# GabrieleConte/pokemon-sprite-generator

Measured on AMD Instinct MI355X. Metric: unet_train_steps_per_sec_bs256, higher is better.
Workload: dtype bf16; 1 GPU; full train_step (add_noise+fwd+SmoothL1+bwd+clip+AdamW), U-Net 640M params, per-GPU batch 256, 27x27x8 latents, 32x256 text, 8 heads, train mode (dropout 0.05), bf16 MFMA / fp32 master+accum; per_gpu_batch=256, global_batch=256, parallelism=dp1

## Files before the change

### include/psg_hip.h

```cpp
#ifndef PSG_HIP_H
#define PSG_HIP_H

#include <stdint.h>

#ifdef __cplusplus
extern "C" {
#endif

typedef void* psg_stream_t;

enum psg_status {
    PSG_OK = 0,
    PSG_ERR_SHAPE = -1,
    PSG_ERR_DTYPE = -2,
    PSG_ERR_ALIGN = -3,
    PSG_ERR_WORKSPACE = -4,
    PSG_ERR_HIP = -5,
    PSG_ERR_ARG = -6
};
enum psg_dtype { PSG_F32 = 0, PSG_BF16 = 1 };
enum psg_act { PSG_ACT_NONE = 0, PSG_ACT_SILU = 1, PSG_ACT_GELU = 2, PSG_ACT_RELU = 3, PSG_ACT_TANH = 4 };
enum psg_flag {
    PSG_FLAG_NOISY_BAD = 1,
    PSG_FLAG_T_RANGE = 2,
    PSG_FLAG_PRED_BAD = 4,
    PSG_FLAG_LOSS_BAD = 8,
    PSG_FLAG_FALLBACK = 16,
    PSG_FLAG_INPUT_BAD = 32,
    PSG_FLAG_SKIP_MASK = 47
};

const char* psg_last_error(void);
int psg_version(void);
// ... 140 lines not shown
int psg_attn_route(int pass, int dtype, int B, int heads, int L, int S, int d, int64_t ldq, int64_t ldk, int64_t ldv,
                   int64_t ldo, int64_t ld_grads, int ptrs_aligned16, int32_t* out);
int psg_attn_bwd(const void* q, int64_t ldq, const void* k, int64_t ldk, const void* v, int64_t ldv,
                 const void* o, int64_t ldo, const void* dout, int64_t lddo, const float* lse,
                 float* delta, void* dq, int64_t lddq, void* dk, int64_t lddk, void* dv, int64_t lddv,
                 int B, int heads, int L, int S, int d, float scale, float drop_p, uint64_t seed,
                 int dtype, psg_stream_t stream);

int psg_attn_bwd_longq(const void* q, int64_t ldq, const void* k, int64_t ldk, const void* v, int64_t ldv,
                       const void* o, int64_t ldo, const void* dout, int64_t lddo, const float* lse,
                       float* delta, void* dq, int64_t lddq, void* dk, int64_t lddk, void* dv, int64_t lddv,
                       int B, int heads, int L, int S, int d, float scale, float drop_p, uint64_t seed,
                       int dtype, void* ws, int64_t ws_bytes, psg_stream_t stream);
int64_t psg_attn_bwd_longq_workspace_bytes(int B, int heads, int L, int S, int d);

int psg_attn_bwd_varlen(const void* q, int64_t ldq, const void* k, int64_t ldk, const void* v, int64_t ldv,
                        const void* o, int64_t ldo, const void* dout, int64_t lddo, const float* lse,
                        float* delta, void* dq, int64_t lddq, void* dk, int64_t lddk, void* dv, int64_t lddv,
                        int B, int heads, int L, int S, int d, float scale, float drop_p, uint64_t seed,
                        int dtype, const int32_t* kv_len, psg_stream_t stream);

int psg_layernorm(const void* x, int64_t ldx, const void* r, int64_t ldr, void* y, int64_t ldy, const float* gamma,
                  const float* beta, int64_t rows, int N, float eps, int x_dtype, int y_dtype, psg_stream_t stream);
int psg_layernorm_bwd(const void* x, int64_t ldx, const void* r, int64_t ldr, const void* dy, int64_t lddy,
                      const float* gamma, void* dz, int64_t lddz, float* dgamma, float* dbeta, int accumulate,
                      int64_t rows, int N, float eps, int x_dtype, int dy_dtype, void* ws, int64_t ws_bytes,
                      psg_stream_t stream);
int64_t psg_layernorm_bwd_workspace_bytes(int64_t rows, int N);
int psg_bert_embed_ln(const int64_t* ids, const int64_t* type_ids, const float* word_emb, const float* pos_emb,
                      const float* type_emb, const float* gamma, const float* beta, void* y, int64_t ldy, int B, int S,
// ... 31 lines not shown
```

### pokemon_sprite_generator_amd/_lib.py

```python
import ctypes as C
import os

import torch

_HERE = os.path.dirname(os.path.abspath(__file__))
LIB_PATH = os.environ.get("PSG_LIB_PATH") or os.path.join(_HERE, "libpsg_hip.so")

PSG_F32, PSG_BF16 = 0, 1
ACT_NONE, ACT_SILU, ACT_GELU, ACT_RELU, ACT_TANH = 0, 1, 2, 3, 4
CONV_SAVE_DACT, CONV_DACT_MUL, CONV_GENERIC_EPILOGUE = 1, 2, 4
FLAG_NOISY_BAD, FLAG_T_RANGE, FLAG_PRED_BAD, FLAG_LOSS_BAD, FLAG_FALLBACK, FLAG_INPUT_BAD, FLAG_SKIP_MASK = 1, 2, 4, 8, 16, 32, 47

c_void_p, c_int, c_int64, c_float, c_uint64 = C.c_void_p, C.c_int, C.c_int64, C.c_float, C.c_uint64


class ConvDesc(C.Structure):
    _fields_ = [
        ("dtype", C.c_int32), ("B", C.c_int32), ("Hi", C.c_int32), ("Wi", C.c_int32), ("Cin", C.c_int32),
        ("Ho", C.c_int32), ("Wo", C.c_int32), ("Cout", C.c_int32),
        ("ksize", C.c_int32), ("stride", C.c_int32), ("pad", C.c_int32),
        ("transposed", C.c_int32), ("act", C.c_int32),
        ("alpha", C.c_float), ("drop_p", C.c_float), ("flags", C.c_int32), ("drop_seed", C.c_uint64),
        ("ldx", C.c_int64), ("ldy", C.c_int64), ("ld_rowadd", C.c_int64), ("ld_residual", C.c_int64),
        ("ld_preact", C.c_int64), ("ld_dact", C.c_int64), ("ldw", C.c_int64),
# ... 60 lines not shown
                                 c_uint64, c_int, c_void_p]),
    "psg_dropout_apply": (c_int, [c_void_p, c_int64, c_void_p, c_int64, c_int64, c_int, c_float, c_uint64, c_float, c_int, c_void_p]),
    "psg_attn_fwd": (c_int, [c_void_p, c_int64, c_void_p, c_int64, c_void_p, c_int64, c_void_p, c_int64, c_void_p]
                     + [c_int] * 5 + [c_float, c_float, c_uint64, c_int, c_void_p]),
    "psg_attn_fwd_varlen": (c_int, [c_void_p, c_int64, c_void_p, c_int64, c_void_p, c_int64, c_void_p, c_int64, c_void_p]
                            + [c_int] * 5 + [c_float, c_float, c_uint64, c_int, c_void_p, c_void_p]),
    "psg_attn_fwd_varlen_train": (c_int, [c_void_p, c_int64, c_void_p, c_int64, c_void_p, c_int64, c_void_p, c_int64, c_void_p]
                                  + [c_int] * 5 + [c_float, c_float, c_uint64, c_int, c_void_p, c_void_p]),
    "psg_attn_bwd_varlen": (c_int, [c_void_p, c_int64] * 5 + [c_void_p, c_void_p] + [c_void_p, c_int64] * 3
                            + [c_int] * 5 + [c_float, c_float, c_uint64, c_int, c_void_p, c_void_p]),
    "psg_attn_path_counts": (c_int, [c_void_p, c_void_p, c_void_p]),
    "psg_attn_set_paths": (c_int, [c_int]),
    "psg_attn_route": (c_int, [c_int] * 7 + [c_int64] * 5 + [c_int, c_void_p]),
    "psg_attn_bwd": (c_int, [c_void_p, c_int64] * 5 + [c_void_p, c_void_p] + [c_void_p, c_int64] * 3
                     + [c_int] * 5 + [c_float, c_float, c_uint64, c_int, c_void_p]),
    "psg_attn_bwd_longq": (c_int, [c_void_p, c_int64] * 5 + [c_void_p, c_void_p] + [c_void_p, c_int64] * 3
                           + [c_int] * 5 + [c_float, c_float, c_uint64, c_int, c_void_p, c_int64, c_void_p]),
    "psg_attn_bwd_longq_workspace_bytes": (c_int64, [c_int] * 5),
    "psg_recon_loss_f32": (c_int, [c_void_p] * 4 + [c_int64, c_float, c_float, c_void_p, c_void_p]),
    "psg_recon_loss_workspace_bytes": (c_int64, []),
    "psg_layernorm": (c_int, [c_void_p, c_int64, c_void_p, c_int64, c_void_p, c_int64, c_void_p, c_void_p, c_int64, c_int, c_float,
                              c_int, c_int, c_void_p]),
    "psg_layernorm_bwd": (c_int, [c_void_p, c_int64, c_void_p, c_int64, c_void_p, c_int64, c_void_p, c_void_p, c_int64, c_void_p, c_void_p,
                                  c_int, c_int64, c_int, c_float, c_int, c_int, c_void_p, c_int64, c_void_p]),
    "psg_layernorm_bwd_workspace_bytes": (c_int64, [c_int64, c_int]),
    "psg_bert_embed_ln": (c_int, [c_void_p] * 8 + [c_int64] + [c_int] * 6 + [c_float, c_int, c_void_p]),
    "psg_sumsq_f32": (c_int, [c_void_p, c_int64, c_void_p, c_int, c_void_p, c_void_p]),
    "psg_adamw_f32": (c_int, [c_void_p] * 4 + [c_int64] + [c_float] * 5 + [c_int, c_void_p, c_float, c_void_p, c_void_p, c_void_p]),
    "psg_adamw_dev_f32": (c_int, [c_void_p] * 4 + [c_int64, c_void_p, c_void_p, c_int] + [c_float] * 4 + [c_void_p, c_void_p, c_float, c_void_p, c_void_p, c_void_p]),
    "psg_clip_scale_f32": (c_int, [c_void_p, c_int64, c_void_p, c_float, c_void_p]),
# ... 146 lines not shown
```

### pokemon_sprite_generator_amd/csrc/attention.h

```cpp
#pragma once
#include "psg_common.h"

namespace psg {

template <typename T>
struct AttnArgs {
    const T *q, *k, *v, *o, *dout;
    T *out, *dq, *dk, *dv;
    float* lse; float* delta;
    int64_t ldq, ldk, ldv, ldo, lddo, lddq, lddk, lddv;
    int B, H, L, S, d;
    float scale;
    uint32_t drop_thresh; float drop_scale; uint64_t seed;
    const uint64_t* seed_dev;
    const int32_t* kv_len;
};

template <typename NDs, typename F>
inline bool with_nd(NDs nds, int d, F&& f) { return d % 16 == 0 && with_const(nds, d / 16, f); }
template <int... NDs, typename F>
inline int for_each_nd(std::integer_sequence<int, NDs...>, F&& f) {
    int rc = PSG_OK;
    ((rc = rc ? rc : f(std::integral_constant<int, NDs>{})), ...);
    return rc;
// ... 3 lines not shown
    int nd;
    int waves;
    int kw, qw, dkv_waves;
    int qw_cut, w_cut;
    int nh, kv_reg;
    size_t lds_fwd, lds_dq, lds_dkv;
    int grid_q[2], grid_kv[2];
};

bool attn_mfma_applicable(int L, int S, int d, int64_t ldq, int64_t ldk, int64_t ldv, int64_t ldo, bool forward_only);
AttnPlan attn_mfma_plan(int B, int H, int L, int S, int d);
int attn_mfma_init_attrs();
template <bool VARLEN> int attn_mfma_fwd(const AttnArgs<bf16_t>& p, hipStream_t s);
template <bool VARLEN> int attn_mfma_bwd(const AttnArgs<bf16_t>& p, hipStream_t s);

bool attn_f32_applicable(int L, int S, int d, int64_t ldq, int64_t ldk, int64_t ldv, int64_t ldo, bool forward_only);
AttnPlan attn_f32_plan(int B, int H, int L, int S, int d);
int attn_f32_init_attrs();
template <bool VARLEN> int attn_f32_fwd(const AttnArgs<float>& p, hipStream_t s);
template <bool VARLEN> int attn_f32_bwd(const AttnArgs<float>& p, hipStream_t s);

int attn_longq_init_attrs();

}
```

### pokemon_sprite_generator_amd/csrc/attention.hip

```cpp
#include "attention.h"
#include <type_traits>

namespace psg {

constexpr int AT_Q = 16;
constexpr int AT_KC = 32;
constexpr int AT_MAXC = 20;

template <typename T>
__device__ __forceinline__ uint64_t attn_idx(const AttnArgs<T>& p, int bh, int l, int s) {
    return ((uint64_t)bh * p.L + l) * (uint64_t)(2 * ((p.S + 1) >> 1)) + s;
}

template <typename T>
__device__ __forceinline__ void stage_rows(float* dst, const T* base, int64_t ld, int r0, int rows, int rmax, int d, float scl) {
    const int d4 = d >> 2;
    for (int e = threadIdx.x; e < rows * d4; e += blockDim.x) {
        const int r = e / d4, c = (e - r * d4) * 4;
        f32x4 v = {0.f, 0.f, 0.f, 0.f};
        if (r0 + r < rmax) v = load4<T>(base + (int64_t)(r0 + r) * ld + c);
        float* o = dst + r * (d + 1) + c;
        o[0] = v[0] * scl; o[1] = v[1] * scl; o[2] = v[2] * scl; o[3] = v[3] * scl;
    }
}
// ... 414 lines not shown
        }
        PSG_LAUNCH_CHECK("attn_bwd");
    } else if (varlen) {
        hipLaunchKernelGGL((attn_fwd_kernel<T, true>), grid, block, pl.lds_fwd, s, p);
        PSG_LAUNCH_CHECK("attn_fwd_varlen");
    } else {
        hipLaunchKernelGGL((attn_fwd_kernel<T, false>), grid, block, pl.lds_fwd, s, p);
        PSG_LAUNCH_CHECK("attn_fwd");
    }
    return PSG_OK;
}

template <typename F>
static int with_elem(int dtype, F&& f) { return dtype == PSG_BF16 ? f((bf16_t*)nullptr) : f((float*)nullptr); }

static int attn_bwd_entry(const char* who, const int32_t* kv_len, const void* q, int64_t ldq, const void* k, int64_t ldk, const void* v, int64_t ldv, const void* o,
                 int64_t ldo, const void* dout, int64_t lddo, const float* lse, float* delta, void* dq, int64_t lddq,
                 void* dk, int64_t lddk, void* dv, int64_t lddv, int B, int heads, int L, int S, int d, float scale,
                 float drop_p, uint64_t seed, int dtype, psg_stream_t stream) {
    PSG_REQUIRE(q && k && v && o && dout && lse && delta && dq && dk && dv, PSG_ERR_ARG, "%s: null pointer", who);
    int rc = attn_check(who, B, heads, L, S, d, dtype, ldq, ldk, ldv, ldo);
    if (rc) return rc;
    PSG_REQUIRE(lddo >= heads * d && lddq >= heads * d && lddk >= heads * d && lddv >= heads * d && ((lddo | lddq | lddk | lddv) & 3) == 0,
                PSG_ERR_SHAPE, "%s: gradient row strides", who);
    PSG_REQUIRE(drop_p >= 0.f && drop_p < 1.f, PSG_ERR_ARG, "%s: drop_p", who);
    rc = attn_check_lds(who, ATTN_BWD, S, d);
    if (rc) return rc;
    return with_elem(dtype, [&](auto* tag) {
        using T = std::remove_pointer_t<decltype(tag)>;
        AttnArgs<T> p = {};
        p.q = (const T*)q; p.k = (const T*)k; p.v = (const T*)v; p.o = (const T*)o; p.dout = (const T*)dout; p.lse = const_cast<float*>(lse); p.delta = delta;
        p.dq = (T*)dq; p.dk = (T*)dk; p.dv = (T*)dv;
        p.ldq = ldq; p.ldk = ldk; p.ldv = ldv; p.ldo = ldo; p.lddo = lddo; p.lddq = lddq; p.lddk = lddk; p.lddv = lddv;
        p.B = B; p.H = heads; p.L = L; p.S = S; p.d = d; p.scale = scale;
        p.drop_thresh = drop_p > 0.f ? drop_thresh(drop_p) : 0u; p.drop_scale = drop_p > 0.f ? 1.0f / (1.0f - drop_p) : 1.0f; p.seed = seed; p.seed_dev = seed_source(); p.kv_len = kv_len;
        return attn_route(kv_len ? ATTN_BWD_VARLEN : ATTN_BWD, p, (hipStream_t)stream);
    });
}

}
using namespace psg;

extern "C" {

int psg_attn_init_attrs(void) {
    { int rc = attn_mfma_init_attrs(); if (rc) return rc; }
    { int rc = attn_f32_init_attrs(); if (rc) return rc; }
    { int rc = attn_longq_init_attrs(); if (rc) return rc; }
    { int rc = valu_init_attrs<float>(); if (rc) return rc; }
    return valu_init_attrs<bf16_t>();
}

// ... 90 lines not shown
                 void* dk, int64_t lddk, void* dv, int64_t lddv, int B, int heads, int L, int S, int d, float scale,
                 float drop_p, uint64_t seed, int dtype, psg_stream_t stream) {
    return attn_bwd_entry("attn_bwd", nullptr, q, ldq, k, ldk, v, ldv, o, ldo, dout, lddo, lse, delta, dq, lddq, dk, lddk, dv, lddv, B, heads, L, S, d,
                          scale, drop_p, seed, dtype, stream);
}

int psg_attn_bwd_varlen(const void* q, int64_t ldq, const void* k, int64_t ldk, const void* v, int64_t ldv, const void* o,
                        int64_t ldo, const void* dout, int64_t lddo, const float* lse, float* delta, void* dq, int64_t lddq,
                        void* dk, int64_t lddk, void* dv, int64_t lddv, int B, int heads, int L, int S, int d, float scale,
                        float drop_p, uint64_t seed, int dtype, const int32_t* kv_len, psg_stream_t stream) {
    PSG_REQUIRE(kv_len, PSG_ERR_ARG, "attn_bwd_varlen: null pointer");
    return attn_bwd_entry("attn_bwd_varlen", kv_len, q, ldq, k, ldk, v, ldv, o, ldo, dout, lddo, lse, delta, dq, lddq, dk, lddk, dv, lddv, B, heads, L, S,
                          d, scale, drop_p, seed, dtype, stream);
}

}
```

### pokemon_sprite_generator_amd/csrc/attention_mfma.hip

```cpp
#include "attention.h"

#ifndef PSG_STAGE_U
#define PSG_STAGE_U 10
#endif
namespace psg {

typedef __attribute__((ext_vector_type(8))) short s16x8;
#define LDS_TR(ptr) __builtin_amdgcn_ds_read_tr16_b64_v4i16((__attribute__((address_space(3))) s16x4*)(ptr))

__device__ __forceinline__ bf16x8 cat_tr(s16x4 a, s16x4 b) {
    s16x8 v = {a[0], a[1], a[2], a[3], b[0], b[1], b[2], b[3]};
    return *reinterpret_cast<bf16x8*>(&v);
}
__device__ __forceinline__ bf16x8 pack8(const f32x16& x, int s2) {
    bf16x8 r;
#pragma unroll
    for (int j = 0; j < 8; ++j) r[j] = (bf16_t)x[8 * s2 + j];
    return r;
}
constexpr bool mfma_kv_reg(int nd) { return nd <= 5; }
constexpr int mfma_nh(int nd) { return nd > 10 ? 2 : 1; }
__device__ __forceinline__ int acc_row(int r, int h) { return (r & 3) + 8 * (r >> 2) + 4 * h; }

__device__ __forceinline__ void stage_tile(char* dst, const bf16_t* src, int64_t ld, int row0, int nrows, int nvalid_end,
                                           int d, int d32, int stride, int tid, int nthreads) {
    const int cpr = d32 >> 3;
    const int n = nrows * cpr;
    constexpr int U = PSG_STAGE_U;
    for (int e0 = tid; e0 < n; e0 += nthreads * U) {
        uint4 v[U];
#pragma unroll
        for (int u = 0; u < U; ++u) {
            const int e = e0 + u * nthreads;
            const int r = e / cpr, c = e - r * cpr;
            const int gr = row0 + r;
            const bool ok = e < n && gr < nvalid_end && c * 8 < d;
            const uint4 t = *reinterpret_cast<const uint4*>(src + (ok ? (int64_t)gr * ld + c * 8 : 0));
            v[u] = ok ? t : make_uint4(0, 0, 0, 0);
        }
#pragma unroll
        for (int u = 0; u < U; ++u) {
            const int e = e0 + u * nthreads;
            const int r = e / cpr, c = e - r * cpr;
// ... 417 lines not shown
                    const int dd = (hp * TH + t) * 32 + 8 * g4 + 4 * fh;
                    if (dd < d) {
                        f32x4 a = {dk[t][4 * g4], dk[t][4 * g4 + 1], dk[t][4 * g4 + 2], dk[t][4 * g4 + 3]};
                        f32x4 c = {dv[t][4 * g4], dv[t][4 * g4 + 1], dv[t][4 * g4 + 2], dv[t][4 * g4 + 3]};
                        if (VARLEN && !kok) { a = f32x4{0.f, 0.f, 0.f, 0.f}; c = a; }
                        store4<bf16_t>(dkg + (int64_t)key * p.lddk + dd, a);
                        store4<bf16_t>(dvg + (int64_t)key * p.lddv + dd, c);
                    }
                }
        }
        }
        __builtin_amdgcn_wave_barrier();
    }
}

using MfmaNDs = std::integer_sequence<int, 1, 2, 4, 5, 10, 20>;
static inline size_t str_bytes(int d) { return 2 * (size_t)d + 16; }
static inline size_t fwd_lds_m(int S, int d) { return 2 * (size_t)((S + 31) & ~31) * str_bytes(d) + 32; }
static inline int attn_waves(int rows) { const int t = (rows + 31) / 32; return t < 1 ? 1 : (t > 4 ? 4 : t); }
constexpr size_t MFMA_LDS_CAP = 158 * 1024;
static inline size_t dkv_lds_w(int L, int d, int waves) {
    const size_t Lp = (L + 31) & ~31;
    return 2 * Lp * str_bytes(d) + 32 + (mfma_kv_reg(d / 16) ? 0 : (size_t)waves * 2 * 32 * str_bytes(d) + 32);
}
struct DkvSplit { int kw, qw, waves; bool qw_cut, w_cut; };
static inline DkvSplit dkv_split(int L, int S, int d) {
    const int nkt = (S + 31) / 32, nqt = (L + 31) / 32;
    int kw = attn_waves(S);
    int qw = 1;
    bool qw_cut = false, w_cut = false;
    if (d <= 80 && nkt <= 2 && kw == nkt) {
// ... 16 lines not shown
    return fwd_lds_m(S, d) <= MFMA_LDS_CAP && (forward_only || dkv_lds_m(L, S, d) <= MFMA_LDS_CAP);
}

AttnPlan attn_mfma_plan(int B, int H, int L, int S, int d) {
    const DkvSplit w = dkv_split(L, S, d);
    AttnPlan pl = {};
    pl.nd = d / 16; pl.waves = attn_waves(L);
    pl.kw = w.kw; pl.qw = w.qw; pl.dkv_waves = w.waves; pl.qw_cut = w.qw_cut; pl.w_cut = w.w_cut;
    pl.nh = mfma_nh(d / 16); pl.kv_reg = mfma_kv_reg(d / 16);
    pl.lds_fwd = pl.lds_dq = fwd_lds_m(S, d); pl.lds_dkv = dkv_lds_w(L, d, w.waves);
    pl.grid_q[0] = pl.grid_kv[0] = B * H; pl.grid_q[1] = pl.grid_kv[1] = 1;
    return pl;
}

int attn_mfma_init_attrs() {
    return for_each_nd(MfmaNDs{}, [](auto nd) {
        constexpr int ND = decltype(nd)::value;
        return set_max_lds((int)MFMA_LDS_CAP, attn_fwd_mfma<ND, false>, attn_fwd_mfma<ND, true>, attn_dq_mfma<ND, false>, attn_dq_mfma<ND, true>,
                           attn_dkv_mfma<ND, false>, attn_dkv_mfma<ND, true>);
    });
}

template <bool VARLEN>
int attn_mfma_fwd(const AttnArgs<bf16_t>& p, hipStream_t s) {
    const AttnPlan pl = attn_mfma_plan(p.B, p.H, p.L, p.S, p.d);
    if (!with_nd(MfmaNDs{}, p.d, [&](auto nd) {
            hipLaunchKernelGGL((attn_fwd_mfma<decltype(nd)::value, VARLEN>), dim3(pl.grid_q[0], pl.grid_q[1]), dim3(64 * pl.waves), pl.lds_fwd, s, p);
        }))
        return set_error(PSG_ERR_SHAPE, "attn_fwd_mfma: head_dim %d", p.d);
    PSG_LAUNCH_CHECK(VARLEN ? "attn_fwd_mfma_varlen" : "attn_fwd_mfma");
    return PSG_OK;
}
template int attn_mfma_fwd<false>(const AttnArgs<bf16_t>&, hipStream_t);
template int attn_mfma_fwd<true>(const AttnArgs<bf16_t>&, hipStream_t);
// ... 3 lines not shown
    const AttnPlan pl = attn_mfma_plan(p.B, p.H, p.L, p.S, p.d);
    if (!with_nd(MfmaNDs{}, p.d, [&](auto nd) {
            hipLaunchKernelGGL((attn_dq_mfma<decltype(nd)::value, VARLEN>), dim3(pl.grid_q[0], pl.grid_q[1]), dim3(64 * pl.waves), pl.lds_dq, s, p);
        }))
        return set_error(PSG_ERR_SHAPE, "attn_dq_mfma: head_dim %d", p.d);
    PSG_LAUNCH_CHECK("attn_dq_mfma");
    with_nd(MfmaNDs{}, p.d, [&](auto nd) {
        hipLaunchKernelGGL((attn_dkv_mfma<decltype(nd)::value, VARLEN>), dim3(pl.grid_kv[0], pl.grid_kv[1]), dim3(64 * pl.dkv_waves), pl.lds_dkv, s, p);
    });
    PSG_LAUNCH_CHECK("attn_dkv_mfma");
    return PSG_OK;
}
template int attn_mfma_bwd<false>(const AttnArgs<bf16_t>&, hipStream_t);
template int attn_mfma_bwd<true>(const AttnArgs<bf16_t>&, hipStream_t);

}
```

### pokemon_sprite_generator_amd/ops.py

```python
import ctypes as C
import os
import struct
import threading

import torch

from . import _lib
from ._lib import ACT_GELU, ACT_NONE, ACT_SILU, ConvDesc, WgradDesc, check, dtype_code, ptr, stream_ptr

__all__ = ["conv2d", "linear", "group_norm", "group_norm_split", "attention_self", "attention_cross", "attention_cross_longq",
           "cross_in_proj", "upsample_bilinear", "nchw_to_nhwc", "nchw_to_nhwc_grad", "nhwc_to_nchw", "image_out", "recon_loss", "text_pool", "timestep_sinusoid", "WeightCache", "ACT_NONE", "ACT_SILU", "ACT_GELU"]


def _lib_for(t):
    if not t.is_cuda:
        raise _lib.PsgError("pokemon_sprite_generator_amd ops need GPU tensors: the HIP kernels are the only implementation")
    return _lib.init(t.device.index if t.device.index is not None else torch.cuda.current_device())


class RowCopies:
    count = 0
    bytes = 0
    warn = os.environ.get("PSG_WARN_COPIES", "0") != "0"

# ... 946 lines not shown
                                    int(gacc if want_g else bacc), rows, N, eps, dtype_code(xr.dtype), dtype_code(dy.dtype), ptr(ws),
                                    ws.numel() if ws is not None else 0, stream_ptr()), "psg_layernorm_bwd")
        if bo2 is not bo:
            bo.add_(bo2) if bacc else bo.copy_(bo2)
        dg = _param_ret(go, ge) if want_g else None
        db = _param_ret(bo, be) if want_b else None
        need_x = ctx.needs_input_grad[0]
        need_r = rr is not None and ctx.needs_input_grad[4]
        return (dz if need_x else None), dg, db, None, (dz if need_r else None), None


def layer_norm(x, weight, bias, eps, residual=None, out_dtype=None):
    return _LayerNormFn.apply(x, weight, bias, eps, residual, out_dtype)


class _AttnFn(torch.autograd.Function):

    @staticmethod
    def forward(ctx, q_src, kv_src, heads, drop_p, seed, kv_len=None):
        lib = _lib_for(q_src)
        dtype = q_src.dtype
        self_mode = kv_src is None
        qr, ldq = _rows(q_src)
        B, L = q_src.shape[0], q_src.shape[1]
        esz = qr.element_size()
        if self_mode:
            E = q_src.shape[-1] // 3
            S = L
            kp, vp, ldk = qr.data_ptr() + E * esz, qr.data_ptr() + 2 * E * esz, ldq
            kvr = None
# ... 27 lines not shown
        dor, lddo = _rows(do)
        esz = qr.element_size()
        delta = torch.empty((B, heads, L), dtype=torch.float32, device=do.device)
        if self_mode:
            dqkv = torch.empty(qshape, dtype=dtype, device=do.device)
            W3 = 3 * E
            kp, vp = qr.data_ptr() + E * esz, qr.data_ptr() + 2 * E * esz
            dqp, dkp, dvp, lddq, lddk = dqkv.data_ptr(), dqkv.data_ptr() + E * esz, dqkv.data_ptr() + 2 * E * esz, W3, W3
            dkv = None
        else:
            dqkv = torch.empty(qshape, dtype=dtype, device=do.device)
            dkv = torch.empty(kvshape, dtype=dtype, device=do.device)
            kp, vp = kvr.data_ptr(), kvr.data_ptr() + E * esz
            dqp, dkp, dvp, lddq, lddk = dqkv.data_ptr(), dkv.data_ptr(), dkv.data_ptr() + E * esz, E, 2 * E
        if ctx.kv_len is None:
            check(lib.psg_attn_bwd(qr.data_ptr(), ldq, kp, ldk, vp, ldk, ptr(o), E, ptr(dor), lddo, ptr(lse), ptr(delta), dqp, lddq, dkp,
                                   lddk, dvp, lddk, B, heads, L, S, d, scale, float(drop_p), int(seed), dtype_code(dtype), stream_ptr()),
                  "psg_attn_bwd")
        else:
            check(lib.psg_attn_bwd_varlen(qr.data_ptr(), ldq, kp, ldk, vp, ldk, ptr(o), E, ptr(dor), lddo, ptr(lse), ptr(delta), dqp, lddq,
                                          dkp, lddk, dvp, lddk, B, heads, L, S, d, scale, float(drop_p), int(seed), dtype_code(dtype),
                                          ptr(ctx.kv_len), stream_ptr()), "psg_attn_bwd_varlen")
        return dqkv, dkv, None, None, None, None


def attention_self(qkv, heads, drop_p=0.0, seed=0, kv_len=None):
    if kv_len is None:
        return _AttnFn.apply(qkv, None, heads, drop_p, seed)
    return _AttnFn.apply(qkv, None, heads, drop_p, seed, kv_len)


def attention_cross(q, kv, heads, drop_p=0.0, seed=0):
    return _AttnFn.apply(q, kv, heads, drop_p, seed)
# ... 195 lines not shown
```

Before: 13.34 bs256-steps/s.

## Add fused single-kernel attention backward for short key sequences

Adds a fused MFMA attention backward kernel that computes delta, dQ, dK and dV in one launch per (batch, head). It keeps K/V (and Q/dO when they fit) in LDS and splits waves across key and query tiles, reducing partial dQ and dK/dV through shared memory. It replaces the separate dq/dkv kernels and delta pass for bf16 cases with S<=64 and head_dim 80 or 160, removing extra launches and re-reads of Q, K, V and dO. The cost is a per-block reduction in LDS and possibly lower occupancy from one block per head. It is on by default and can be disabled with an environment variable.

```diff
diff --git a/include/psg_hip.h b/include/psg_hip.h
--- a/include/psg_hip.h
+++ b/include/psg_hip.h
@@ -16,7 +16,8 @@
     PSG_ERR_ALIGN = -3,
     PSG_ERR_WORKSPACE = -4,
     PSG_ERR_HIP = -5,
-    PSG_ERR_ARG = -6
+    PSG_ERR_ARG = -6,
+    PSG_ERR_NOT_APPLICABLE = -7
 };
 enum psg_dtype { PSG_F32 = 0, PSG_BF16 = 1 };
 enum psg_act { PSG_ACT_NONE = 0, PSG_ACT_SILU = 1, PSG_ACT_GELU = 2, PSG_ACT_RELU = 3, PSG_ACT_TANH = 4 };
@@ -187,6 +188,17 @@
                        int dtype, void* ws, int64_t ws_bytes, psg_stream_t stream);
 int64_t psg_attn_bwd_longq_workspace_bytes(int B, int heads, int L, int S, int d);
 
+int psg_attn_bwd_fused(const void* q, int64_t ldq, const void* k, int64_t ldk, const void* v, int64_t ldv,
+                       const void* o, int64_t ldo, const void* dout, int64_t lddo, const float* lse,
+                       float* delta, void* dq, int64_t lddq, void* dk, int64_t lddk, void* dv, int64_t lddv,
+                       int B, int heads, int L, int S, int d, float scale, float drop_p, uint64_t seed,
+                       int dtype, psg_stream_t stream);
+#define PSG_ATTN_FUSED_FIELDS 6
+int psg_attn_bwd_fused_applicable(int dtype, int B, int heads, int L, int S, int d, int64_t ldq, int64_t ldk, int64_t ldv,
+                                  int64_t ldo, int64_t ld_grads, int32_t* out);
+int psg_attn_set_bwd_fused(int on);
+int psg_attn_get_bwd_fused(void);
+
 int psg_attn_bwd_varlen(const void* q, int64_t ldq, const void* k, int64_t ldk, const void* v, int64_t ldv,
                         const void* o, int64_t ldo, const void* dout, int64_t lddo, const float* lse,
                         float* delta, void* dq, int64_t lddq, void* dk, int64_t lddk, void* dv, int64_t lddv,
diff --git a/pokemon_sprite_generator_amd/_lib.py b/pokemon_sprite_generator_amd/_lib.py
--- a/pokemon_sprite_generator_amd/_lib.py
+++ b/pokemon_sprite_generator_amd/_lib.py
@@ -98,6 +98,11 @@
     "psg_attn_route": (c_int, [c_int] * 7 + [c_int64] * 5 + [c_int, c_void_p]),
     "psg_attn_bwd": (c_int, [c_void_p, c_int64] * 5 + [c_void_p, c_void_p] + [c_void_p, c_int64] * 3
                      + [c_int] * 5 + [c_float, c_float, c_uint64, c_int, c_void_p]),
+    "psg_attn_bwd_fused": (c_int, [c_void_p, c_int64] * 5 + [c_void_p, c_void_p] + [c_void_p, c_int64] * 3
+                           + [c_int] * 5 + [c_float, c_float, c_uint64, c_int, c_void_p]),
+    "psg_attn_bwd_fused_applicable": (c_int, [c_int] * 6 + [c_int64] * 5 + [c_void_p]),
+    "psg_attn_set_bwd_fused": (c_int, [c_int]),
+    "psg_attn_get_bwd_fused": (c_int, []),
     "psg_attn_bwd_longq": (c_int, [c_void_p, c_int64] * 5 + [c_void_p, c_void_p] + [c_void_p, c_int64] * 3
                            + [c_int] * 5 + [c_float, c_float, c_uint64, c_int, c_void_p, c_int64, c_void_p]),
     "psg_attn_bwd_longq_workspace_bytes": (c_int64, [c_int] * 5),
diff --git a/pokemon_sprite_generator_amd/csrc/attention.h b/pokemon_sprite_generator_amd/csrc/attention.h
--- a/pokemon_sprite_generator_amd/csrc/attention.h
+++ b/pokemon_sprite_generator_amd/csrc/attention.h
@@ -41,6 +41,10 @@
 template <bool VARLEN> int attn_mfma_fwd(const AttnArgs<bf16_t>& p, hipStream_t s);
 template <bool VARLEN> int attn_mfma_bwd(const AttnArgs<bf16_t>& p, hipStream_t s);
 
+struct AttnFusedPlan { int waves, kw, qw; bool priv; size_t lds; };
+bool attn_fused_plan(int L, int S, int d, int64_t ldq, int64_t ldk, int64_t ldv, int64_t ldo, int64_t ldg, AttnFusedPlan* out);
+int attn_fused_bwd(const AttnArgs<bf16_t>& p, hipStream_t s);
+
 bool attn_f32_applicable(int L, int S, int d, int64_t ldq, int64_t ldk, int64_t ldv, int64_t ldo, bool forward_only);
 AttnPlan attn_f32_plan(int B, int H, int L, int S, int d);
 int attn_f32_init_attrs();
diff --git a/pokemon_sprite_generator_amd/csrc/attention.hip b/pokemon_sprite_generator_amd/csrc/attention.hip
--- a/pokemon_sprite_generator_amd/csrc/attention.hip
+++ b/pokemon_sprite_generator_amd/csrc/attention.hip
@@ -452,28 +452,49 @@
 template <typename F>
 static int with_elem(int dtype, F&& f) { return dtype == PSG_BF16 ? f((bf16_t*)nullptr) : f((float*)nullptr); }
 
+static int attn_bwd_check(const char* who, const void* q, int64_t ldq, const void* k, int64_t ldk, const void* v, int64_t ldv, const void* o, int64_t ldo,
+                          const void* dout, int64_t lddo, const float* lse, float* delta, void* dq, int64_t lddq, void* dk, int64_t lddk, void* dv,
+                          int64_t lddv, int B, int heads, int L, int S, int d, float drop_p, int dtype) {
+    PSG_REQUIRE(q && k && v && o && dout && lse && delta && dq && dk && dv, PSG_ERR_ARG, "%s: null pointer", who);
+    int rc = attn_check(who, B, heads, L, S, d, dtype, ldq, ldk, ldv, ldo);
+    if (rc) return rc;
+    PSG_REQUIRE(lddo >= heads * d && lddq >= heads * d && lddk >= heads * d && lddv >= heads * d && ((lddo | lddq | lddk | lddv) & 3) == 0,
+                PSG_ERR_SHAPE, "%s: gradient row strides", who);
+    PSG_REQUIRE(drop_p >= 0.f && drop_p < 1.f, PSG_ERR_ARG, "%s: drop_p", who);
+    return attn_check_lds(who, ATTN_BWD, S, d);
+}
+
+template <typename T>
+static AttnArgs<T> attn_bwd_args(const int32_t* kv_len, const void* q, int64_t ldq, const void* k, int64_t ldk, const void* v, int64_t ldv, const void* o,
+                                 int64_t ldo, const void* dout, int64_t lddo, const float* lse, float* delta, void* dq, int64_t lddq, void* dk,
+                                 int64_t lddk, void* dv, int64_t lddv, int B, int heads, int L, int S, int d, float scale, float drop_p, uint64_t seed) {
+    AttnArgs<T> p = {};
+    p.q = (const T*)q; p.k = (const T*)k; p.v = (const T*)v; p.o = (const T*)o; p.dout = (const T*)dout; p.lse = const_cast<float*>(lse); p.delta = delta;
+    p.dq = (T*)dq; p.dk = (T*)dk; p.dv = (T*)dv;
+    p.ldq = ldq; p.ldk = ldk; p.ldv = ldv; p.ldo = ldo; p.lddo = lddo; p.lddq = lddq; p.lddk = lddk; p.lddv = lddv;
+    p.B = B; p.H = heads; p.L = L; p.S = S; p.d = d; p.scale = scale;
+    p.drop_thresh = drop_p > 0.f ? drop_thresh(drop_p) : 0u; p.drop_scale = drop_p > 0.f ? 1.0f / (1.0f - drop_p) : 1.0f; p.seed = seed; p.seed_dev = seed_source(); p.kv_len = kv_len;
+    return p;
+}
+
 static int attn_bwd_entry(const char* who, const int32_t* kv_len, const void* q, int64_t ldq, const void* k, int64_t ldk, const void* v, int64_t ldv, const void* o,
                  int64_t ldo, const void* dout, int64_t lddo, const float* lse, float* delta, void* dq, int64_t lddq,
                  void* dk, int64_t lddk, void* dv, int64_t lddv, int B, int heads, int L, int S, int d, float scale,
                  float drop_p, uint64_t seed, int dtype, psg_stream_t stream) {
-    PSG_REQUIRE(q && k && v && o && dout && lse && delta && dq && dk && dv, PSG_ERR_ARG, "%s: null pointer", who);
-    int rc = attn_check(who, B, heads, L, S, d, dtype, ldq, ldk, ldv, ldo);
-    if (rc) return rc;
-    PSG_REQUIRE(lddo >= heads * d && lddq >= heads * d && lddk >= heads * d && lddv >= heads * d && ((lddo | lddq | lddk | lddv) & 3) == 0,
-                PSG_ERR_SHAPE, "%s: gradient row strides", who);
-    PSG_REQUIRE(drop_p >= 0.f && drop_p < 1.f, PSG_ERR_ARG, "%s: drop_p", who);
-    rc = attn_check_lds(who, ATTN_BWD, S, d);
+    const int rc = attn_bwd_check(who, q, ldq, k, ldk, v, ldv, o, ldo, dout, lddo, lse, delta, dq, lddq, dk, lddk, dv, lddv, B, heads, L, S, d, drop_p, dtype);
     if (rc) return rc;
     return with_elem(dtype, [&](auto* tag) {
         using T = std::remove_pointer_t<decltype(tag)>;
-        AttnArgs<T> p = {};
-        p.q = (const T*)q; p.k = (const T*)k; p.v = (const T*)v; p.o = (const T*)o; p.dout = (const T*)dout; p.lse = const_cast<float*>(lse); p.delta = delta;
-        p.dq = (T*)dq; p.dk = (T*)dk; p.dv = (T*)dv;
-        p.ldq = ldq; p.ldk = ldk; p.ldv = ldv; p.ldo = ldo; p.lddo = lddo; p.lddq = lddq; p.lddk = lddk; p.lddv = lddv;
-        p.B = B; p.H = heads; p.L = L; p.S = S; p.d = d; p.scale = scale;
-        p.drop_thresh = drop_p > 0.f ? drop_thresh(drop_p) : 0u; p.drop_scale = drop_p > 0.f ? 1.0f / (1.0f - drop_p) : 1.0f; p.seed = seed; p.seed_dev = seed_source(); p.kv_len = kv_len;
+        const AttnArgs<T> p = attn_bwd_args<T>(kv_len, q, ldq, k, ldk, v, ldv, o, ldo, dout, lddo, lse, delta, dq, lddq, dk, lddk, dv, lddv, B, heads, L, S, d,
+                                               scale, drop_p, seed);
         return attn_route(kv_len ? ATTN_BWD_VARLEN : ATTN_BWD, p, (hipStream_t)stream);
     });
+}
+
+static int g_bwd_fused = -1;
+static int bwd_fused_on() {
+    if (g_bwd_fused < 0) { const char* e = getenv("PSG_ATTN_BWD_FUSED"); g_bwd_fused = (e && atoi(e) == 0) ? 0 : 1; }
+    return g_bwd_fused;
 }
 
 }
@@ -594,4 +615,41 @@
                           d, scale, drop_p, seed, dtype, stream);
 }
 
-}
+int psg_attn_bwd_fused(const void* q, int64_t ldq, const void* k, int64_t ldk, const void* v, int64_t ldv, const void* o,
+                       int64_t ldo, const void* dout, int64_t lddo, const float* lse, float* delta, void* dq, int64_t lddq,
+                       void* dk, int64_t lddk, void* dv, int64_t lddv, int B, int heads, int L, int S, int d, float scale,
+                       float drop_p, uint64_t seed, int dtype, psg_stream_t stream) {
+    const char* who = "attn_bwd_fused";
+    const int rc = attn_bwd_check(who, q, ldq, k, ldk, v, ldv, o, ldo, dout, lddo, lse, delta, dq, lddq, dk, lddk, dv, lddv, B, heads, L, S, d, drop_p, dtype);
+    if (rc) return rc;
+    const bool ptrs_ok = aligned16(q) && aligned16(k) && aligned16(v) && aligned16(o) && aligned16(dout) && aligned8(dq) && aligned8(dk) && aligned8(dv);
+    if (dtype != PSG_BF16 || !ptrs_ok || !attn_fused_plan(L, S, d, ldq, ldk, ldv, ldo, lddo | lddq | lddk | lddv, nullptr))
+        return set_error(PSG_ERR_NOT_APPLICABLE, "%s: not a fused call (dtype %d, L=%d S=%d head_dim=%d, strides or pointer alignment)", who, dtype, L, S, d);
+    const AttnArgs<bf16_t> p = attn_bwd_args<bf16_t>(nullptr, q, ldq, k, ldk, v, ldv, o, ldo, dout, lddo, lse, delta, dq, lddq, dk, lddk, dv, lddv, B, heads, L,
+                                                     S, d, scale, drop_p, seed);
+    ProfScope prof(PROF_ATTN, 10.0 * (double)B * heads * L * S * d, (hipStream_t)stream, (double)B * heads * d * (4.0 * L + 4.0 * S) * (double)sizeof(bf16_t));
+    ++g_attn_paths[ATTN_MFMA_BF16];
+    return attn_fused_bwd(p, (hipStream_t)stream);
+}
+
+int psg_attn_bwd_fused_applicable(int dtype, int B, int heads, int L, int S, int d, int64_t ldq, int64_t ldk, int64_t ldv, int64_t ldo,
+                                  int64_t ld_grads, int32_t* out) {
+    const char* who = "attn_bwd_fused_applicable";
+    PSG_REQUIRE(out, PSG_ERR_ARG, "%s: null pointer", who);
+    int rc = attn_check(who, B, heads, L, S, d, dtype, ldq, ldk, ldv, ldo);
+    if (rc) return rc;
+    PSG_REQUIRE(ld_grads >= heads * d && (ld_grads & 3) == 0, PSG_ERR_SHAPE, "%s: gradient row strides", who);
+    rc = attn_check_lds(who, ATTN_BWD, S, d);
+    if (rc) return rc;
+    AttnFusedPlan pl = {};
+    const bool taken = dtype == PSG_BF16 && attn_fused_plan(L, S, d, ldq, ldk, ldv, ldo, ld_grads, &pl);
+    const int32_t v[PSG_ATTN_FUSED_FIELDS] = {taken ? 1 : 0, taken ? pl.waves : 0, taken ? pl.kw : 0, taken ? pl.qw : 0, taken ? (int32_t)pl.lds : 0,
+                                              taken ? B * heads : 0};
+    for (int i = 0; i < PSG_ATTN_FUSED_FIELDS; ++i) out[i] = v[i];
+    return PSG_OK;
+}
+
+int psg_attn_set_bwd_fused(int on) { g_bwd_fused = on ? 1 : 0; return PSG_OK; }
+int psg_attn_get_bwd_fused(void) { return bwd_fused_on(); }
+
+}
diff --git a/pokemon_sprite_generator_amd/csrc/attention_mfma.hip b/pokemon_sprite_generator_amd/csrc/attention_mfma.hip
--- a/pokemon_sprite_generator_amd/csrc/attention_mfma.hip
+++ b/pokemon_sprite_generator_amd/csrc/attention_mfma.hip
@@ -1,4 +1,5 @@
 #include "attention.h"
+#include <algorithm>
 
 #ifndef PSG_STAGE_U
 #define PSG_STAGE_U 10
@@ -22,11 +23,11 @@
 constexpr int mfma_nh(int nd) { return nd > 10 ? 2 : 1; }
 __device__ __forceinline__ int acc_row(int r, int h) { return (r & 3) + 8 * (r >> 2) + 4 * h; }
 
+template <int U = PSG_STAGE_U>
 __device__ __forceinline__ void stage_tile(char* dst, const bf16_t* src, int64_t ld, int row0, int nrows, int nvalid_end,
                                            int d, int d32, int stride, int tid, int nthreads) {
     const int cpr = d32 >> 3;
     const int n = nrows * cpr;
-    constexpr int U = PSG_STAGE_U;
     for (int e0 = tid; e0 < n; e0 += nthreads * U) {
         uint4 v[U];
 #pragma unroll
@@ -474,7 +475,239 @@
     }
 }
 
+constexpr int FUSED_TSTR = 64;
+template <int ND, bool PRIV>
+__global__ __launch_bounds__(256, (ND <= 5 ? 2 : 1)) void attn_bwd_fused_mfma(const AttnArgs<bf16_t> p) {
+    constexpr int NDT = (ND + 1) / 2;
+    constexpr int STR = 2 * ND * 16 + 16;
+    constexpr int TSTR = FUSED_TSTR;
+    extern __shared__ __attribute__((aligned(16))) char smem[];
+    const int Lp = (p.L + 31) & ~31, Sp = (p.S + 31) & ~31;
+    const int W = (int)(blockDim.x >> 6);
+    const int QGrows = PRIV ? W * 32 : Lp;
+    char* Qs = smem;
+    char* Gs = Qs + QGrows * STR;
+    char* Ks = Gs + QGrows * STR;
+    char* Vs = Ks + Sp * STR;
+    char* Tall = Vs + Sp * STR + 32;
+    float* dqp = reinterpret_cast<float*>(Tall + W * 32 * TSTR);
+    const int bh = blockIdx.x, b = bh / p.H, hd = bh - b * p.H;
+    const uint64_t seed = eff_seed(p.seed, p.drop_thresh ? p.seed_dev : nullptr);
+    const int d = ND * 16;
+    const int tid = threadIdx.x, lane = tid & 63, wave = tid >> 6;
+    const bf16_t* qg = p.q + (int64_t)b * p.L * p.ldq + hd * d;
+    const bf16_t* kg = p.k + (int64_t)b * p.S * p.ldk + hd * d;
+    const bf16_t* vg = p.v + (int64_t)b * p.S * p.ldv + hd * d;
+    const bf16_t* gg = p.dout + (int64_t)b * p.L * p.lddo + hd * d;
+    const bf16_t* og = p.o + (int64_t)b * p.L * p.ldo + hd * d;
+    bf16_t* dqg = p.dq + (int64_t)b * p.L * p.lddq + hd * d;
+    bf16_t* dkg = p.dk + (int64_t)b * p.S * p.lddk + hd * d;
+    bf16_t* dvg = p.dv + (int64_t)b * p.S * p.lddv + hd * d;
+    stage_tile(Ks, kg, p.ldk, 0, Sp, p.S, d, d, STR, tid, (int)blockDim.x);
+    stage_tile(Vs, vg, p.ldv, 0, Sp, p.S, d, d, STR, tid, (int)blockDim.x);
+    if (!PRIV) {
+        stage_tile(Qs, qg, p.ldq, 0, Lp, p.L, d, d, STR, tid, (int)blockDim.x);
+        stage_tile(Gs, gg, p.lddo, 0, Lp, p.L, d, d, STR, tid, (int)blockDim.x);
+    }
+    const int fr = lane & 31, fh = lane >> 5;
+    auto delta_tile = [&](int rt, char* Qt) {
+        const int l = rt * 32 + fr;
+        const bool lok = l < p.L;
+        const int ls = lok ? l : 0;
+        float del = 0.f;
+#pragma unroll
+        for (int ks = 0; ks < ND; ++ks) {
+            uint4 w = *reinterpret_cast<const uint4*>(gg + (int64_t)ls * p.lddo + 16 * ks + 8 * fh);
+            const uint4 ov = *reinterpret_cast<const uint4*>(og + (int64_t)ls * p.ldo + 16 * ks + 8 * fh);
+            if (!lok) w = make_uint4(0, 0, 0, 0);
+            const bf16x8 gf = *reinterpret_cast<const bf16x8*>(&w), of = *reinterpret_cast<const bf16x8*>(&ov);
+#pragma unroll
+            for (int j = 0; j < 8; ++j) del += (float)gf[j] * (float)of[j];
+        }
+        del += __shfl_xor(del, 32, 64);
+        if (!lok) del = 0.f;
+        if (fh == 0) {
+            float* pad = reinterpret_cast<float*>(Qt + fr * STR + 2 * d);
+            pad[0] = lok ? p.lse[(int64_t)bh * p.L + ls] : 0.f;
+            pad[1] = del;
+            if (lok) p.delta[(int64_t)bh * p.L + l] = del;
+        }
+    };
+    if (!PRIV)
+        for (int rt = wave; rt * 32 < Lp; rt += W) delta_tile(rt, Qs + rt * 32 * STR);
+    __syncthreads();
+
+    const int nqt = Lp >> 5;
+    const int KW = Sp >> 5, QW = W / KW;
+    const int kw = wave % KW, qw = wave / KW;
+    const int key = kw * 32 + fr;
+    const bool kok = key < p.S;
+    char* Tw = Tall + wave * (32 * TSTR);
+    f32x16 dk[NDT], dv[NDT];
+#pragma unroll
+    for (int t = 0; t < NDT; ++t)
+#pragma unroll
+        for (int e = 0; e < 16; ++e) { dk[t][e] = 0.f; dv[t][e] = 0.f; }
+    const int niter = (nqt + QW - 1) / QW;
+    for (int it = 0; it < niter; ++it) {
+        const int qt = qw + it * QW;
+        const bool live = qt < nqt;
+        f32x16 dq[NDT];
+        char* Qt = PRIV ? Qs + wave * 32 * STR : Qs + qt * 32 * STR;
+        char* Gt = PRIV ? Gs + wave * 32 * STR : Gs + qt * 32 * STR;
+        if (PRIV && live) {
+            stage_tile<ND>(Qt, qg, p.ldq, qt * 32, 32, p.L, d, d, STR, lane, 64);
+            stage_tile<ND>(Gt, gg, p.lddo, qt * 32, 32, p.L, d, d, STR, lane, 64);
+            delta_tile(qt, Qt);
+            __atomic_signal_fence(__ATOMIC_SEQ_CST);
+            __builtin_amdgcn_wave_barrier();
+        }
+        if (live) {
+            f32x16 st, dp;
+#pragma unroll
+            for (int e = 0; e < 16; ++e) { st[e] = 0.f; dp[e] = 0.f; }
+#pragma unroll
+            for (int ks = 0; ks < ND; ++ks) {
+                const int co = (16 * ks + 8 * fh) * 2;
+                const bf16x8 qa = *reinterpret_cast<const bf16x8*>(Qt + fr * STR + co);
+                const bf16x8 ga = *reinterpret_cast<const bf16x8*>(Gt + fr * STR + co);
+                const bf16x8 kb = *reinterpret_cast<const bf16x8*>(Ks + key * STR + co);
+                const bf16x8 vb = *reinterpret_cast<const bf16x8*>(Vs + key * STR + co);
+                st = __builtin_amdgcn_mfma_f32_32x32x16_bf16(qa, kb, st, 0, 0, 0);
+                dp = __builtin_amdgcn_mfma_f32_32x32x16_bf16(ga, vb, dp, 0, 0, 0);
+            }
+            f32x16 pd;
+            const uint32_t hS = (uint32_t)((p.S + 1) >> 1), koff = (uint32_t)(key >> 1);
+            const DropRow dr = drop_row(seed, ((uint64_t)bh * p.L + (uint64_t)(qt * 32)) * (uint64_t)hS);
+            const uint32_t t16 = p.drop_thresh >> 16;
+            const int odd = key & 1, hsh = odd ? 16 : 0;
+            uint32_t hmine[8], hpeer[8];
+            if (p.drop_thresh) {
+#pragma unroll
+                for (int j = 0; j < 8; ++j) {
+                    hmine[j] = drop_hash_row(dr, (uint32_t)(acc_row(j, fh) + 16 * odd) * hS + koff);
+                    hpeer[j] = (uint32_t)__builtin_amdgcn_mov_dpp((int)hmine[j], 0xB1, 0xF, 0xF, false);
+                }
+            }
+#pragma unroll
+            for (int r = 0; r < 16; ++r) {
+                const float2 ld2 = *reinterpret_cast<const float2*>(Qt + acc_row(r, fh) * STR + 2 * d);
+                const float pr = __expf(st[r] * p.scale - ld2.x);
+                float dpr = dp[r], pv = pr;
+                if (p.drop_thresh) {
+                    const uint32_t hh = ((r >> 3) == odd) ? hmine[r & 7] : hpeer[r & 7];
+                    const bool keep = ((hh >> hsh) & 0xFFFFu) >= t16;
+                    pv = keep ? pr * p.drop_scale : 0.f;
+                    dpr = keep ? dpr * p.drop_scale : 0.f;
+                }
+                pd[r] = pv; st[r] = pr * (dpr - ld2.y) * p.scale;
+            }
+            const bf16x8 pf0 = pack8(pd, 0), pf1 = pack8(pd, 1), sf0 = pack8(st, 0), sf1 = pack8(st, 1);
+            {
+                const uint4 s0 = *reinterpret_cast<const uint4*>(&sf0), s1 = *reinterpret_cast<const uint4*>(&sf1);
+                char* trow = Tw + fr * TSTR + 8 * fh;
+                *reinterpret_cast<uint2*>(trow) = make_uint2(s0.x, s0.y);
+                *reinterpret_cast<uint2*>(trow + 16) = make_uint2(s0.z, s0.w);
+                *reinterpret_cast<uint2*>(trow + 32) = make_uint2(s1.x, s1.y);
+                *reinterpret_cast<uint2*>(trow + 48) = make_uint2(s1.z, s1.w);
+            }
+            __atomic_signal_fence(__ATOMIC_SEQ_CST);
+            __builtin_amdgcn_wave_barrier();
+#pragma unroll
+            for (int t = 0; t < NDT; ++t) {
+                const bf16x8 g0 = tr_frag(Gt, STR, 0, 0, t * 32, lane);
+                const bf16x8 g1 = tr_frag(Gt, STR, 0, 1, t * 32, lane);
+                dv[t] = __builtin_amdgcn_mfma_f32_32x32x16_bf16(g0, pf0, dv[t], 0, 0, 0);
+                dv[t] = __builtin_amdgcn_mfma_f32_32x32x16_bf16(g1, pf1, dv[t], 0, 0, 0);
+                const bf16x8 q0 = tr_frag(Qt, STR, 0, 0, t * 32, lane);
+                const bf16x8 q1 = tr_frag(Qt, STR, 0, 1, t * 32, lane);
+                dk[t] = __builtin_amdgcn_mfma_f32_32x32x16_bf16(q0, sf0, dk[t], 0, 0, 0);
+                dk[t] = __builtin_amdgcn_mfma_f32_32x32x16_bf16(q1, sf1, dk[t], 0, 0, 0);
+            }
+            const bf16x8 b0 = tr_frag(Tw, TSTR, 0, 0, 0, lane);
+            const bf16x8 b1 = tr_frag(Tw, TSTR, 0, 1, 0, lane);
+            __atomic_signal_fence(__ATOMIC_SEQ_CST);
+            __builtin_amdgcn_wave_barrier();
+#pragma unroll
+            for (int t = 0; t < NDT; ++t) {
+#pragma unroll
+                for (int e = 0; e < 16; ++e) dq[t][e] = 0.f;
+                const bf16x8 k0 = tr_frag(Ks, STR, kw * 32, 0, t * 32, lane);
+                const bf16x8 k1 = tr_frag(Ks, STR, kw * 32, 1, t * 32, lane);
+                dq[t] = __builtin_amdgcn_mfma_f32_32x32x16_bf16(k0, b0, dq[t], 0, 0, 0);
+                dq[t] = __builtin_amdgcn_mfma_f32_32x32x16_bf16(k1, b1, dq[t], 0, 0, 0);
+            }
+        }
+        if (KW > 1) {
+            float* slot = dqp + (int64_t)qw * (NDT * 16 * 64) + lane;
+            if (live && kw == 1) {
+#pragma unroll
+                for (int t = 0; t < NDT; ++t)
+#pragma unroll
+                    for (int e = 0; e < 16; ++e) slot[(t * 16 + e) * 64] = dq[t][e];
+            }
+            __syncthreads();
+            if (live && kw == 0) {
+#pragma unroll
+                for (int t = 0; t < NDT; ++t)
+#pragma unroll
+                    for (int e = 0; e < 16; ++e) dq[t][e] += slot[(t * 16 + e) * 64];
+            }
+            if (it + 1 < niter) __syncthreads();
+        }
+        const int l = qt * 32 + fr;
+        if (live && kw == 0 && l < p.L) {
+#pragma unroll
+            for (int t = 0; t < NDT; ++t)
+#pragma unroll
+                for (int g4 = 0; g4 < 4; ++g4) {
+                    const int dd = t * 32 + 8 * g4 + 4 * fh;
+                    if (dd < d) {
+                        f32x4 v = {dq[t][4 * g4], dq[t][4 * g4 + 1], dq[t][4 * g4 + 2], dq[t][4 * g4 + 3]};
+                        store4<bf16_t>(dqg + (int64_t)l * p.lddq + dd, v);
+                    }
+                }
+        }
+    }
+    if (QW > 1) {
+        __syncthreads();
+        float* red = reinterpret_cast<float*>(smem);
+        if (qw > 0) {
+            float* dst = red + (int64_t)((qw - 1) * KW + kw) * (NDT * 2 * 16 * 64) + lane;
+#pragma unroll
+            for (int t = 0; t < NDT; ++t)
+#pragma unroll
+                for (int e = 0; e < 16; ++e) { dst[((t * 2) * 16 + e) * 64] = dk[t][e]; dst[((t * 2 + 1) * 16 + e) * 64] = dv[t][e]; }
+        }
+        __syncthreads();
+        if (qw == 0) {
+            for (int q2 = 1; q2 < QW; ++q2) {
+                const float* src = red + (int64_t)((q2 - 1) * KW + kw) * (NDT * 2 * 16 * 64) + lane;
+#pragma unroll
+                for (int t = 0; t < NDT; ++t)
+#pragma unroll
+                    for (int e = 0; e < 16; ++e) { dk[t][e] += src[((t * 2) * 16 + e) * 64]; dv[t][e] += src[((t * 2 + 1) * 16 + e) * 64]; }
+            }
+        }
+    }
+    if (kok && qw == 0) {
+#pragma unroll
+        for (int t = 0; t < NDT; ++t)
+#pragma unroll
+            for (int g4 = 0; g4 < 4; ++g4) {
+                const int dd = t * 32 + 8 * g4 + 4 * fh;
+                if (dd < d) {
+                    f32x4 a = {dk[t][4 * g4], dk[t][4 * g4 + 1], dk[t][4 * g4 + 2], dk[t][4 * g4 + 3]};
+                    f32x4 c = {dv[t][4 * g4], dv[t][4 * g4 + 1], dv[t][4 * g4 + 2], dv[t][4 * g4 + 3]};
+                    store4<bf16_t>(dkg + (int64_t)key * p.lddk + dd, a);
+                    store4<bf16_t>(dvg + (int64_t)key * p.lddv + dd, c);
+                }
+            }
+    }
+}
+
 using MfmaNDs = std::integer_sequence<int, 1, 2, 4, 5, 10, 20>;
+using FusedNDs = std::integer_sequence<int, 5, 10>;
 static inline size_t str_bytes(int d) { return 2 * (size_t)d + 16; }
 static inline size_t fwd_lds_m(int S, int d) { return 2 * (size_t)((S + 31) & ~31) * str_bytes(d) + 32; }
 static inline int attn_waves(int rows) { const int t = (rows + 31) / 32; return t < 1 ? 1 : (t > 4 ? 4 : t); }
@@ -521,10 +754,14 @@
 }
 
 int attn_mfma_init_attrs() {
-    return for_each_nd(MfmaNDs{}, [](auto nd) {
+    const int rc = for_each_nd(MfmaNDs{}, [](auto nd) {
         constexpr int ND = decltype(nd)::value;
         return set_max_lds((int)MFMA_LDS_CAP, attn_fwd_mfma<ND, false>, attn_fwd_mfma<ND, true>, attn_dq_mfma<ND, false>, attn_dq_mfma<ND, true>,
                            attn_dkv_mfma<ND, false>, attn_dkv_mfma<ND, true>);
+    });
+    if (rc) return rc;
+    return for_each_nd(FusedNDs{}, [](auto nd) {
+        return set_max_lds((int)MFMA_LDS_CAP, attn_bwd_fused_mfma<decltype(nd)::value, false>, attn_bwd_fused_mfma<decltype(nd)::value, true>);
     });
 }
 
@@ -558,4 +795,32 @@
 template int attn_mfma_bwd<false>(const AttnArgs<bf16_t>&, hipStream_t);
 template int attn_mfma_bwd<true>(const AttnArgs<bf16_t>&, hipStream_t);
 
-}
+bool attn_fused_plan(int L, int S, int d, int64_t ldq, int64_t ldk, int64_t ldv, int64_t ldo, int64_t ldg, AttnFusedPlan* out) {
+    if (!with_nd(FusedNDs{}, d, [](auto) {})) return false;
+    if (((ldq | ldk | ldv | ldo | ldg) & 7) != 0) return false;
+    if (L < 1 || S < 1 || S > 64) return false;
+    const int nkt = (S + 31) / 32, nqt = (L + 31) / 32, ndt = (d / 16 + 1) / 2;
+    const int kw = nkt, qw = std::min(4 / kw, nqt), waves = kw * qw;
+    const bool priv = kw == 1 && nqt > qw;
+    const size_t images = 2 * (size_t)((priv ? waves : nqt) + nkt) * 32 * str_bytes(d) + 32;
+    const size_t live = images + (size_t)waves * 32 * FUSED_TSTR + (kw > 1 ? (size_t)qw * ndt * 16 * 64 * sizeof(float) : 0);
+    const size_t red = (size_t)(qw - 1) * kw * ndt * 2 * 16 * 64 * sizeof(float);
+    const size_t lds = std::max(live, red);
+    if (lds > MFMA_LDS_CAP) return false;
+    if (out) { out->waves = waves; out->kw = kw; out->qw = qw; out->priv = priv; out->lds = lds; }
+    return true;
+}
+
+int attn_fused_bwd(const AttnArgs<bf16_t>& p, hipStream_t s) {
+    AttnFusedPlan pl;
+    if (!attn_fused_plan(p.L, p.S, p.d, p.ldq, p.ldk, p.ldv, p.ldo, p.lddo | p.lddq | p.lddk | p.lddv, &pl))
+        return set_error(PSG_ERR_NOT_APPLICABLE, "attn_bwd_fused: L=%d S=%d head_dim=%d is not a fused shape", p.L, p.S, p.d);
+    with_nd(FusedNDs{}, p.d, [&](auto nd) {
+        if (pl.priv) hipLaunchKernelGGL((attn_bwd_fused_mfma<decltype(nd)::value, true>), dim3(p.B * p.H), dim3(64 * pl.waves), pl.lds, s, p);
+        else hipLaunchKernelGGL((attn_bwd_fused_mfma<decltype(nd)::value, false>), dim3(p.B * p.H), dim3(64 * pl.waves), pl.lds, s, p);
+    });
+    PSG_LAUNCH_CHECK("attn_bwd_fused_mfma");
+    return PSG_OK;
+}
+
+}
diff --git a/pokemon_sprite_generator_amd/ops.py b/pokemon_sprite_generator_amd/ops.py
--- a/pokemon_sprite_generator_amd/ops.py
+++ b/pokemon_sprite_generator_amd/ops.py
@@ -984,6 +984,19 @@
     return _LayerNormFn.apply(x, weight, bias, eps, residual, out_dtype)
 
 
+_ATTN_BWD_FUSED = {}
+
+
+def _attn_bwd_fused_taken(lib, dtype, B, heads, L, S, d, ldq, ldk, ldo, ldg):
+    key = (dtype, B, heads, L, S, d, ldq, ldk, ldo, ldg)
+    taken = _ATTN_BWD_FUSED.get(key)
+    if taken is None:
+        out = (C.c_int32 * 6)()
+        rc = lib.psg_attn_bwd_fused_applicable(dtype_code(dtype), B, heads, L, S, d, ldq, ldk, ldk, ldo, ldg, C.cast(out, C.c_void_p))
+        taken = _ATTN_BWD_FUSED[key] = rc == 0 and out[0] == 1
+    return taken
+
+
 class _AttnFn(torch.autograd.Function):
 
     @staticmethod
@@ -1041,9 +1054,13 @@
             kp, vp = kvr.data_ptr(), kvr.data_ptr() + E * esz
             dqp, dkp, dvp, lddq, lddk = dqkv.data_ptr(), dkv.data_ptr(), dkv.data_ptr() + E * esz, E, 2 * E
         if ctx.kv_len is None:
-            check(lib.psg_attn_bwd(qr.data_ptr(), ldq, kp, ldk, vp, ldk, ptr(o), E, ptr(dor), lddo, ptr(lse), ptr(delta), dqp, lddq, dkp,
-                                   lddk, dvp, lddk, B, heads, L, S, d, scale, float(drop_p), int(seed), dtype_code(dtype), stream_ptr()),
-                  "psg_attn_bwd")
+            args = (qr.data_ptr(), ldq, kp, ldk, vp, ldk, ptr(o), E, ptr(dor), lddo, ptr(lse), ptr(delta), dqp, lddq, dkp,
+                    lddk, dvp, lddk, B, heads, L, S, d, scale, float(drop_p), int(seed), dtype_code(dtype), stream_ptr())
+            aligned = not any(a & 15 for a in (qr.data_ptr(), kp, vp, o.data_ptr(), dor.data_ptr(), dqp, dkp, dvp))
+            if aligned and lib.psg_attn_get_bwd_fused() and _attn_bwd_fused_taken(lib, dtype, B, heads, L, S, d, ldq, ldk, E, lddo | lddq | lddk):
+                check(lib.psg_attn_bwd_fused(*args), "psg_attn_bwd_fused")
+            else:
+                check(lib.psg_attn_bwd(*args), "psg_attn_bwd")
         else:
             check(lib.psg_attn_bwd_varlen(qr.data_ptr(), ldq, kp, ldk, vp, ldk, ptr(o), E, ptr(dor), lddo, ptr(lse), ptr(delta), dqp, lddq,
                                           dkp, lddk, dvp, lddk, B, heads, L, S, d, scale, float(drop_p), int(seed), dtype_code(dtype),
```

New measurement: 13.43 bs256-steps/s, median of 6. No clear change (+0.7%).
